# rrwick/Badread

Hardware: NVIDIA H100
Metric: simulated Gbases/sec (higher is better)
Workload: dtype u8/int32 (+f64 identity estimate)

## Files before the change

### badread_b200/csrc/bb_api.cu

```cuda
#include <cuda_runtime.h>
#include <dlfcn.h>
#include <unistd.h>

#include <algorithm>
#include <cstdio>
#include <cstdlib>
#include <cstring>
#include <memory>
#include <numeric>
#include <string>
#include <thread>
#include <vector>

#include "bb_kernels.cuh"
#include "bb_launch.h"

namespace {

struct DevBuf {
    void *p = nullptr;
    size_t cap = 0;
    DevBuf() = default;
    DevBuf(const DevBuf &) = delete;
    DevBuf &operator=(const DevBuf &) = delete;
// ... 640 lines not shown
    p.tbuf = w.s_tbuf.as<uint8_t>(); p.tbuf_stride = tbuf_stride;
    p.peq = w.s_peq.as<uint4>(); p.peq_stride = peq_cap; p.peq_cap = peq_cap;
    constexpr int lean_cap = 2048;
    const size_t lean_warps = (size_t)w.ctx->sm_count * kLeanCtasPerSmBoth * BB_WARPS_PER_CTA;
    BB_CUDA(&w, w.s_lr_lean.ensure(lean_warps * lean_cap * 2 * sizeof(int)));
    w.pool_lean = p;
    w.pool_lean.lr = w.s_lr_lean.as<int>(); w.pool_lean.lr_stride = 2ll * lean_cap; w.pool_lean.lr_cap = lean_cap;
    return BB_OK;
}

static BBBatchDev batch_dev(const Worker &w) {
    BBBatchDev B{};
    B.n_reads = w.n_reads;
    B.read_index = w.d_read_index.as<unsigned long long>();
    B.seg_off = w.d_seg_off.as<int>();
    B.segs = w.d_segs.as<bb_segment>();
    B.lit = w.d_lit.as<uint8_t>();
    B.target = w.d_target.as<double>();
    B.order = w.d_order.as<int>();
    B.reads = w.d_reads.as<BBReadDev>();
    B.frag = w.d_frag.as<uint8_t>();
    B.state = w.d_state.as<uint32_t>();
    B.kidx = w.d_kidx.as<int>();
    B.seq = w.d_seq.as<uint8_t>();
    B.ops = w.d_ops.as<uint8_t>();
    B.dcnt = w.d_dcnt.as<unsigned int>();
    B.qual = w.d_qual.as<uint8_t>();
    B.out_seq = w.d_out_seq.as<uint8_t>();
    B.out_qual = w.d_out_qual.as<uint8_t>();
    B.fpeq = w.d_fpeq.as<uint4>();
    B.speq = w.d_speq.as<uint4>();
    B.ctime = w.d_ctime.as<unsigned int>();
    B.chlog = w.d_chlog.as<uint2>();
    B.wres = w.d_wres.as<int2>();
    return B;
}

#define BB_N_COUNTERS 256
#define BB_ROUND_BASE(r) (16 + 16 * (r))
enum { BBC_MUTATE = 0, BBC_NTASKS = 1, BBC_LANE4 = 2, BBC_FB1 = 3, BBC_LANE8 = 4, BBC_FB2 = 5, BBC_WARP = 6, BBC_PENDING = 7 };

static int level_bound(int max_len, double slack) {
    long long mm = (long long)(max_len * slack) + 64;
    int d = 0;
    while (20ll * ((2 * mm + 64 + 63) / 64) * mm + 8ll * mm >= 1048576ll) { mm = (mm + 1) / 2; d++; }
    return d + 1;
}

static int w_prepare(Worker &w) {
    const bb_ctx &c = *w.ctx;
    BB_CUDA(&w, cudaSetDevice(c.device));
    Worker::Layout &L = w.L;
    const int n = w.n_reads;
    const int64_t off = w.frag_total;
    w.seq_cap = (int64_t)((double)off * w.slack) + 16ll * n + 65536;
    w.out_cap = w.seq_cap;
    w.speq_cap = w.seq_cap / 32 + (2ll * BB_PEQ_PAD + 2) * n + 64;
    L.fb_len = w.wres_total + 8;
    BB_CUDA(&w, w.d_frag.ensure((size_t)off + 16));
    BB_CUDA(&w, w.d_state.ensure(((size_t)off + 16) * sizeof(uint32_t)));
    BB_CUDA(&w, w.d_kidx.ensure(((size_t)off + 16) * sizeof(int)));
    BB_CUDA(&w, w.d_counter.ensure(BB_N_COUNTERS * sizeof(int)));
    BB_CUDA(&w, w.d_scan.ensure(sizeof(BBScanOut)));
    BB_CUDA(&w, w.d_levels.ensure(sizeof(Worker::RunInfo::levels)));
    BB_CUDA(&w, w.d_fpeq.ensure(((size_t)w.fpeq_total + 4) * sizeof(uint4)));
    BB_CUDA(&w, w.d_ctime.ensure(((size_t)off + 16) * sizeof(unsigned int)));
    BB_CUDA(&w, w.d_chlog.ensure(((size_t)w.log_total + 16) * sizeof(uint2)));
    BB_CUDA(&w, w.d_wres.ensure(((size_t)w.wres_total + 16) * sizeof(int2)));
    BB_CUDA(&w, w.d_wtasks.ensure(((size_t)w.wres_total + 16) * sizeof(BBWinTask)));
    BB_CUDA(&w, w.d_wfallback.ensure(2 * (size_t)L.fb_len * sizeof(BBWinTask)));
    BB_CUDA(&w, w.d_seq.ensure((size_t)w.seq_cap + 16));
    BB_CUDA(&w, w.d_ops.ensure((size_t)w.seq_cap + 16));
    BB_CUDA(&w, w.d_dcnt.ensure(((size_t)w.seq_cap + 16) * sizeof(unsigned int)));
    BB_CUDA(&w, w.d_qual.ensure((size_t)w.seq_cap + 16));
    BB_CUDA(&w, w.d_speq.ensure(((size_t)w.speq_cap + 4) * sizeof(uint4)));
    BB_CUDA(&w, w.d_out_seq.ensure((size_t)w.out_cap + 16));
    BB_CUDA(&w, w.d_out_qual.ensure((size_t)w.out_cap + 16));
    L.lane_ctas = c.sm_count * 4;
    const size_t lanes = (size_t)L.lane_ctas * 64;
    if (c.knobs.lowmem) {
        L.hist_per_pipe = lanes * BB_LEAF_MAX_TILES * BB_LEAF_CKPT_WORDS;
        BB_CUDA(&w, w.s_leafhist.ensure(2 * L.hist_per_pipe * sizeof(uint32_t)));
    } else {
        L.hist_per_pipe = lanes * BB_LEAF_LANE_COLS * BB_LEAF_LW;
        BB_CUDA(&w, w.s_lanehist.ensure(2 * L.hist_per_pipe * sizeof(uint2)));
    }
    BB_CUDA(&w, w.s_ltbuf.ensure(2 * lanes * BB_WIN_MAX_COLS));
    if (c.knobs.lowmem) BB_CUDA(&w, w.s_wckpt.ensure(2 * lanes * BB_WIN_MAX_TILES * BB_WIN_CKPT_WORDS(BB_WIN_LW) * sizeof(uint32_t)));
    const int len_b = (int)std::min<double>((double)w.max_len * w.slack + 64.0, (double)(1 << 24));
    const int lr_floor = c.knobs.lr_cap > 0 ? c.knobs.lr_cap : 4096;
    int lr_need = lr_floor;
    for (int r = 0; r < n; r++) {
        const double len = (double)w.h_reads[(size_t)r].frag_len;
        const double worst = len * w.slack + 64.0;
        const double expect = c.knobs.lr_cap > 0 ? 0.0 : 3.0 * (1.0 - w.h_target[(size_t)r]) * len + 0.02 * len + 512.0;
        lr_need = std::max(lr_need, (int)std::min(worst, w.lr_worst ? worst : expect));
    }
    int rc = ensure_scratch(w, len_b, lr_need, len_b, lr_floor);
    if (rc) return rc;
    int slot = 0;
    for (int s = 0; s < 2; s++)
        for (int k = 0; k < 3; k++) {
            L.lean_base[s][k] = slot;
            slot += c.sm_count * kLeanCtasPerSm[k] * BB_WARPS_PER_CTA;
        }
    L.cap_node = (int)std::min<int64_t>(w.seq_cap / 256 + 4ll * n + 1024, 0x7ffffff0);
    for (int s = 0; s < 2; s++) {
        auto &qb = w.qbuf[s];
        for (int k = 0; k < BBQ_NODE_CLASSES; k++)
            for (int p = 0; p < 2; p++) BB_CUDA(&w, qb.node[k][p].ensure((size_t)L.cap_node * sizeof(BBNode)));
        for (int x = 0; x < 2; x++) BB_CUDA(&w, qb.leaf[x].ensure((size_t)L.cap_node * sizeof(BBNode)));
        BB_CUDA(&w, qb.count.ensure(kQueueCounts * sizeof(int)));
    }
    w.n_levels = std::max(1, std::min(BB_MAX_LEVELS, level_bound(w.max_len, w.slack) + w.extra_levels));
    return BB_OK;
}

static int check_batch(bb_ctx *ctx, int32_t n_reads, const int32_t *seg_off, const bb_segment *segs, int64_t literal_len,
                       std::vector<int64_t> &len) {
    const int k = ctx->em.k;
    len.assign((size_t)n_reads, 0);
    for (int32_t r = 0; r < n_reads; r++) {
        if (seg_off[r + 1] < seg_off[r]) return set_err(ctx, BB_ERR_ARG, "seg_off must be non-decreasing");
        for (int32_t s = seg_off[r]; s < seg_off[r + 1]; s++) {
            const bb_segment &sg = segs[s];
            if (sg.len < 0 || sg.src < 0) return set_err(ctx, BB_ERR_ARG, "negative segment");
            if (sg.kind == BB_SEG_LITERAL) { if (sg.src + sg.len > literal_len) return set_err(ctx, BB_ERR_ARG, "literal segment out of range"); }
            else if (sg.kind == BB_SEG_REF_FWD || sg.kind == BB_SEG_REF_REV) { if (sg.src + sg.len > ctx->ref_len) return set_err(ctx, BB_ERR_ARG, "reference segment out of range"); }
            else return set_err(ctx, BB_ERR_ARG, "unknown segment kind");
            len[(size_t)r] += sg.len;
        }
        if (len[(size_t)r] + 2 * k >= (1 << 24)) return set_err(ctx, BB_ERR_ARG, "fragment too long (16 Mb limit)");
    }
    return BB_OK;
}

static int w_batch_upload(Worker &w, int32_t n_reads, const uint64_t *read_index, const int32_t *seg_off,
                          const bb_segment *segs, const uint8_t *literal_pool, int64_t literal_len,
                          const double *target_identity) {
    BB_CUDA(&w, cudaSetDevice(w.ctx->device));
    const int k = w.ctx->em.k;
    w.h_reads.assign((size_t)n_reads, BBReadDev{});
    w.h_inlen.assign((size_t)n_reads, 0);
    w.h_target.assign(target_identity, target_identity + n_reads);
    int64_t off = 0, peq_off = 0, log_off = 0, wres_off = 0;
    int max_len = 0;
    for (int32_t r = 0; r < n_reads; r++) {
        int64_t len = 0;
        for (int32_t s = seg_off[r]; s < seg_off[r + 1]; s++) len += segs[s].len;
        w.h_inlen[(size_t)r] = (int32_t)len;
        BBReadDev &rd = w.h_reads[(size_t)r];
        rd.frag_off = off;
        rd.frag_len = (int)(len + 2 * k);
        rd.fpeq_off = peq_off;
        peq_off += bb_peq_words(rd.frag_len);
        {
            const int cap = (int)(0.9 * (double)rd.frag_len) + k + 2;
            rd.log_off = log_off; rd.wres_off = wres_off;
            log_off += cap; wres_off += cap / BB_ALIGNMENT_INTERVAL + 1;
            const double need = (double)rd.frag_len * (1.0 - target_identity[r]);
            rd.horizon = (int)std::min<double>((double)cap, std::max(0.0, 1.25 * need) + 48.0);
            rd.n_logged = 0; rd.n_resume = 0; rd.a_done = 0; rd.status = BB_READ_PENDING; rd.stop_reason = 0;
        }
        off += (rd.frag_len + 15) & ~15;
        max_len = std::max(max_len, rd.frag_len);
    }
    w.frag_total = off; w.fpeq_total = peq_off; w.log_total = log_off; w.wres_total = wres_off;
// ... 1024 lines not shown
```

### badread_b200/csrc/bb_lane.cuh

```cuda
#pragma once
#include <cstdint>

#include "bb_align.cuh"

struct BBLaneProb {
    const uint4 *peq;
    int peq_bit0;
    const uint8_t *q;
    int n;
    const uint8_t *t;
    int m;
    int a, b;
    uint2 *hist;
};

__device__ __forceinline__ int bb_lane_words(int a, int b) { return ((a + b) >> 5) + 2; }

__device__ __forceinline__ void bb_lane_fetch(const BBLaneProb &P, int word, uint32_t &mA, uint32_t &mC, uint32_t &mG,
                                              uint32_t &mT) {
    mA = mC = mG = mT = 0u;
    const int R = word * 32;
    const int valid = P.n - R;
    if (valid <= 0) return;
    const int s = P.peq_bit0 + R;
    const int idx = s >> 5, sh = s & 31;
    const uint4 lo = P.peq[idx], hi = P.peq[idx + 1];
    mA = __funnelshift_r(lo.x, hi.x, sh); mC = __funnelshift_r(lo.y, hi.y, sh);
    mG = __funnelshift_r(lo.z, hi.z, sh); mT = __funnelshift_r(lo.w, hi.w, sh);
    if (valid < 32) {
        const uint32_t keep = (1u << valid) - 1u;
        mA &= keep; mC &= keep; mG &= keep; mT &= keep;
    }
}

template <int LW>
__device__ int bb_lane_pass(const BBLaneProb &P) {
    const int n = P.n, m = P.m, a = P.a;
    uint32_t Pv[LW], Mv[LW], eA[LW], eC[LW], eG[LW], eT[LW];
#pragma unroll
    for (int x = 0; x < LW; x++) {
        Pv[x] = ~0u; Mv[x] = 0u;
        bb_lane_fetch(P, x, eA[x], eC[x], eG[x], eT[x]);
    }
    int wt = 0;
    int score = 32 * LW;
    uint2 *h = P.hist;
    for (int c = 0; c < m; c++) {
        if (c - a >= 32 * (wt + 1)) {
#pragma unroll
            for (int x = 0; x + 1 < LW; x++) {
                Pv[x] = Pv[x + 1]; Mv[x] = Mv[x + 1];
                eA[x] = eA[x + 1]; eC[x] = eC[x + 1]; eG[x] = eG[x + 1]; eT[x] = eT[x + 1];
            }
            wt++;
            Pv[LW - 1] = ~0u; Mv[LW - 1] = 0u;
            bb_lane_fetch(P, wt + LW - 1, eA[LW - 1], eC[LW - 1], eG[LW - 1], eT[LW - 1]);
            score += 32;
        }
        const uint32_t tc = P.t[c];
        const uint32_t code = (tc >> 1) & 3u;
        const bool acgt = ((0x47544341u >> (8 * code)) & 0xffu) == tc;
        uint32_t Eq[LW], Xv[LW], A[LW], S[LW], Ph[LW], Mh[LW];
#pragma unroll
        for (int x = 0; x < LW; x++)
            Eq[x] = (code & 2u) ? ((code & 1u) ? eG[x] : eT[x]) : ((code & 1u) ? eC[x] : eA[x]);
        if (!acgt) {
#pragma unroll
            for (int x = 0; x < LW; x++) {
                Eq[x] = 0u;
                const int row0 = (wt + x) * 32;
                for (int r = 0; r < 32; r++)
                    if (row0 + r < n && P.q[row0 + r] == tc) Eq[x] |= 1u << r;
            }
        }
#pragma unroll
        for (int x = 0; x < LW; x++) { Xv[x] = Eq[x] | Mv[x]; A[x] = Eq[x] & Pv[x]; }
        bb_add_words<LW>(A, Pv, S);
#pragma unroll
        for (int x = 0; x < LW; x++) {
            const uint32_t Xh = (S[x] ^ Pv[x]) | Eq[x];
            Ph[x] = Mv[x] | ~(Xh | Pv[x]);
            Mh[x] = Pv[x] & Xh;
        }
        score += (int)(Ph[LW - 1] >> 31) - (int)(Mh[LW - 1] >> 31);
#pragma unroll
        for (int x = LW - 1; x >= 0; x--) {
            const uint32_t phs = __funnelshift_l(x > 0 ? Ph[x - 1] : 0x80000000u, Ph[x], 1);
            const uint32_t mhs = __funnelshift_l(x > 0 ? Mh[x - 1] : 0u, Mh[x], 1);
            const uint32_t raw = Ph[x];
            Pv[x] = mhs | ~(Xv[x] | phs);
            Mv[x] = phs & Xv[x];
            h[x] = make_uint2(Pv[x], raw);
        }
        h += LW;
    }
    int result = BB_INF;
    int run = score;
#pragma unroll
    for (int x = LW - 1; x >= 0; x--) {
        const int row0 = (wt + x) * 32;
        if (row0 <= n - 1 && n - 1 < row0 + 32) {
            const int bit = (n - 1) - row0;
            const uint32_t up = bit == 31 ? 0u : (Pv[x] >> (bit + 1));
            const uint32_t um = bit == 31 ? 0u : (Mv[x] >> (bit + 1));
            result = run - __popc(up) + __popc(um);
        }
        run -= __popc(Pv[x]) - __popc(Mv[x]);
    }
    return result;
}

template <int LW>
__device__ void bb_lane_traceback(const BBLaneProb &P, int &matches, int &dels, int &err) {
    const int a = P.a;
    int i = P.n - 1, j = P.m - 1;
    int mt = 0, dl = 0;
    while (i >= 0 && j >= 0) {
        int wt = (j - a) >> 5; if (wt < 0) wt = 0;
        const int x = (i >> 5) - wt;
        if (x < 0 || x >= LW) { err |= 1; break; }
        const uint2 e = P.hist[j * LW + x];
        const int bit = i & 31;
        if ((e.x >> bit) & 1u) { i--; }
        else if ((e.y >> bit) & 1u) { dl++; j--; }
        else { mt += (P.q[i] == P.t[j]) ? 1 : 0; i--; j--; }
    }
    if (j >= 0) dl += j + 1;
    matches = mt; dels = dl;
}

template <int LW>
__device__ __forceinline__ void bb_prefetch_history(const uint2 *hist, int tj) {
#if defined(__CUDA_ARCH__)
    const long long e = (long long)tj * LW;
    if ((e & 15) == 0 && e >= 48) asm volatile("prefetch.global.L2 [%0];" ::"l"(hist + (e - 48)));
#endif
}

#define BB_RING_BYTES(LW, T) (2 * (T) * (LW) * 64 * 8)

__device__ __forceinline__ void bb_cp_async8(uint2 *smem, const uint2 *gmem) {
#if defined(__CUDA_ARCH__)
    asm volatile("cp.async.ca.shared.global [%0], [%1], 8;" ::"r"((uint32_t)__cvta_generic_to_shared(smem)), "l"(gmem) : "memory");
#else
    *smem = *gmem;
#endif
}
__device__ __forceinline__ void bb_cp_async_commit() {
#if defined(__CUDA_ARCH__)
    asm volatile("cp.async.commit_group;" ::: "memory");
#endif
}
template <int N>
__device__ __forceinline__ void bb_cp_async_wait() {
#if defined(__CUDA_ARCH__)
    asm volatile("cp.async.wait_group %0;" ::"n"(N) : "memory");
#endif
}

template <int LW, int T>
__device__ __forceinline__ void bb_ring_tick(uint2 *ring, const uint2 *hist, int tj, int &staged_lo) {
    const bool fresh = staged_lo > tj;
    if (fresh) {
        const int lo1 = max(0, tj - T + 1);
        for (int col = tj; col >= lo1; col--) {
#pragma unroll
            for (int x = 0; x < LW; x++) bb_cp_async8(ring + ((col & (2 * T - 1)) * LW + x) * 64, hist + (long long)col * LW + x);
        }
        bb_cp_async_commit();
        staged_lo = lo1;
    }
    const int want_lo = max(0, tj - 2 * T + 1);
    for (int col = staged_lo - 1; col >= want_lo; col--) {
#pragma unroll
        for (int x = 0; x < LW; x++) bb_cp_async8(ring + ((col & (2 * T - 1)) * LW + x) * 64, hist + (long long)col * LW + x);
    }
    bb_cp_async_commit();
    if (want_lo < staged_lo) staged_lo = want_lo;
#if defined(__CUDA_ARCH__)
    {
        constexpr int LINES = (T * LW * 8 + 127) / 128 + 1;
        const long long e = ((long long)tj - 4 * T) * LW;
#pragma unroll
        for (int x = 0; x < 2 * LINES; x++)
            if (e + 16 * x >= 0 && (x < LINES || fresh)) asm volatile("prefetch.global.L2 [%0];" ::"l"(hist + e + 16 * x));
    }
#endif
    bb_cp_async_wait<1>();
}

template <int LW, int T>
__device__ __forceinline__ uint2 bb_ring_entry(const uint2 *ring, int col, int x) {
    return ring[((col & (2 * T - 1)) * LW + x) * 64];
}
```

### badread_b200/csrc/bb_loop.cuh

```cuda
#pragma once
#include <cstdint>

#include "bb_lane.cuh"

enum { BB_STOP_HORIZON = 0, BB_STOP_LIMIT = 1, BB_STOP_COUNT = 2, BB_STOP_NOLOOP = 3 };

#define BB_WIN_LW 8
#define BB_WIN_MAX_COLS 2048

struct BBWinTask { int r, a; };

#define BB_MUTP_THREADS (BB_WARPS_PER_CTA * 32 + 32)

template <int BB_TU_ = 0>
__global__ void __launch_bounds__(BB_MUTP_THREADS)
bb_k_mutate(BBBatchDev B, BBErrorModelDev em, unsigned long long seed, int *work_counter, const int *order,
                 int n_items) {
    constexpr int NE = BB_WARPS_PER_CTA * 32;
    __shared__ int s_kind[2][NE], s_pos[2][NE], s_rpos[2][NE];
    __shared__ uint32_t s_pay[2][NE];
    __shared__ int s_w, s_stop, s_cc;
    __shared__ long long s_n0;
    const int lane = threadIdx.x & 31;
    const int warp = threadIdx.x >> 5;
// ... 343 lines not shown
            if (tm > BB_WIN_MAX_COLS || bb_lane_words(P.a, P.b) > LW || !bb_uses_traceback(qn, tm)) {
                fallback[atomicAdd(fallback_count, 1)] = tk;
                active = false;
            }
        }
        if (!active) tm = 0;
        BBLanePass<LW> S;
        if (active) {
            P.n = qn; P.peq = B.fpeq + rd->fpeq_off; P.q = frag + qpos; P.qs = 1;
            P.peq_bit0 = qpos + BB_PEQ_BIT0; P.t = tbuf; P.ts = 1;
            bb_lane_begin<LW>(S, P);
        }
        const int tm_max = __reduce_max_sync(BB_FULL, tm);
        for (int c = 0; c < tm_max; c++) {
            if (c < tm) {
                if ((c & (BB_WIN_TILE - 1)) == 0) {
                    uint32_t *ck = ckpt + (c / BB_WIN_TILE) * CKW;
#pragma unroll
                    for (int x = 0; x < LW; x++) { ck[x] = S.Pv[x]; ck[LW + x] = S.Mv[x]; }
                    ck[2 * LW] = (uint32_t)S.wt; ck[2 * LW + 1] = (uint32_t)S.score;
                }
                bb_lane_step<LW, false>(S, P, nullptr);
            }
        }
        int ti = qn - 1, tj = tm - 1, matches = 0, dels = 0;
        bool walking = active && ti >= 0 && tj >= 0;
        bool need_tile = walking;
        int tile_lo = 0;
        for (int round = 0; round < 2 * BB_WIN_MAX_COLS + 64 && __any_sync(BB_FULL, walking); round++) {
            if (walking && need_tile) {
                const int tile = tj / BB_WIN_TILE;
                tile_lo = tile * BB_WIN_TILE;
                const uint32_t *ck = ckpt + tile * CKW;
#pragma unroll
                for (int x = 0; x < LW; x++) { S.Pv[x] = ck[x]; S.Mv[x] = ck[LW + x]; }
                S.wt = (int)ck[2 * LW]; S.score = (int)ck[2 * LW + 1]; S.c = tile_lo;
#pragma unroll
                for (int x = 0; x < LW; x++) bb_fetch_peq(P, 32 * (S.wt + x), S.eA[x], S.eC[x], S.eG[x], S.eT[x]);
                const int hi = min(tile_lo + BB_WIN_TILE, tm);
                for (int c = tile_lo; c < hi; c++) bb_lane_step<LW, true, 64>(S, P, hs + ((c - tile_lo) * LW) * 64);
                need_tile = false;
            }
            for (int mv = 0; mv < 64; mv++) {
                const bool can = walking && !need_tile;
                if (!__any_sync(BB_FULL, can)) break;
                if (can) {
                    int wt = (tj - P.a) >> 5; if (wt < 0) wt = 0;
                    const int x = (ti >> 5) - wt;
                    if (x < 0 || x >= LW) { atomicOr(&B.reads[tk.r].flags, 1); ti = -1; tj = -1; }
                    else {
                        const uint2 e = hs[((tj - tile_lo) * LW + x) * 64];
                        const int bit = ti & 31;
                        if ((e.x >> bit) & 1u) ti--;
                        else if ((e.y >> bit) & 1u) { dels++; tj--; }
                        else { matches += (frag[qpos + ti] == tbuf[tj]) ? 1 : 0; ti--; tj--; }
                    }
                    if (ti < 0 || tj < 0) walking = false;
                    else if (tj < tile_lo) need_tile = true;
                }
            }
        }
        if (active) {
            if (walking) atomicOr(&B.reads[tk.r].flags, 1);
            if (tj >= 0) dels += tj + 1;
            B.wres[rd->wres_off + tk.a - 1] = make_int2(matches, qn + dels);
        }
    }
}

#ifndef BB_WIN_RING_T
#define BB_WIN_RING_T 4
#endif
template <int LW, int T = BB_WIN_RING_T>
__global__ void __launch_bounds__(64, (LW <= 4 ? 8 : 4))
bb_k_window_lane_hist(BBBatchDev B, BBErrorModelDev em, const BBWinTask *tasks, const int *n_tasks_ptr, unsigned long long seed,
                 uint2 *hist_pool, uint8_t *tbuf_pool, int *cursor, BBWinTask *fallback, int *fallback_count) {
#ifdef BB_EMULATOR
    static uint2 s_ring[BB_RING_BYTES(LW, T) / 8];
#else
    extern __shared__ __align__(16) uint2 s_ring[];
#endif
    const int n_tasks = *n_tasks_ptr;
    const long long gl = (long long)blockIdx.x * blockDim.x + threadIdx.x;
    uint2 *const hist = hist_pool + gl * (long long)(BB_WIN_MAX_COLS * LW);
    uint8_t *const tbuf = tbuf_pool + gl * (long long)BB_WIN_MAX_COLS;
    uint2 *const ring = s_ring + threadIdx.x;
    BBLanePass<LW> S;
    BBProb P;
    BBWinTask tk = {0, 0};
    const uint8_t *frag = nullptr;
    const uint32_t *state = nullptr;
    const unsigned int *ctime = nullptr;
    int phase = 0;
    int qpos = 0, qn = 0, jx = 0, tm = 0, uw = 0, ti = 0, tj = 0, diags = 0, dels = 0, dist = 0, staged_lo = 0;
    unsigned int tmax = 0;
    for (;;) {
        if (phase == 0) {
            const int w = atomicAdd(cursor, 1);
            if (w >= n_tasks) phase = 4;
            else {
                tk = tasks[w];
                const BBReadDev *rd = &B.reads[tk.r];
                frag = B.frag + rd->frag_off; state = B.state + rd->frag_off; ctime = B.ctime + rd->frag_off;
                bb_window_of(rd->frag_len, seed, B.read_index[tk.r], tk.a, qpos, qn);
                tmax = (unsigned int)(BB_ALIGNMENT_INTERVAL * tk.a);
                jx = 0; tm = 0; uw = 0;
                phase = 1;
            }
        }
        if (__all_sync(BB_FULL, phase == 4)) break;
        for (int it = 0; it < 64; it++) {
            if (phase == 1) {
                unsigned int ct4[4];
                uint8_t fb4[4];
#pragma unroll
                for (int h = 0; h < 4; h++) {
                    const int j = min(jx + h, qn - 1);
                    ct4[h] = ctime[qpos + j];
                    fb4[h] = frag[qpos + j];
                }
#pragma unroll
                for (int h = 0; h < 4; h++) {
                    if (jx < qn) {
                        if (ct4[h] == 0u || ct4[h] > tmax) { if (tm < BB_WIN_MAX_COLS) tbuf[tm] = fb4[h]; tm++; }
                        else {
                            const uint32_t st = state[qpos + jx];
                            const int sl = (int)(st & 0xff);
                            for (int c = 0; c < sl; c++) { if (tm < BB_WIN_MAX_COLS) tbuf[tm] = bb_slot_char(em, st, c); tm++; }
                            uw += sl < 1 ? 1 : sl;
                        }
                        jx++;
                    }
                }
                if (jx >= qn) {
                    const int diff = qn > tm ? qn - tm : tm - qn;
                    if (uw < diff) uw = diff;
                    const int mx = qn > tm ? qn : tm;
                    if (uw > mx) uw = mx;
                    bb_band(qn, tm, uw, P.a, P.b);
                    if (tm > BB_WIN_MAX_COLS || bb_lane_words(P.a, P.b) > LW || !bb_uses_traceback(qn, tm)) {
                        fallback[atomicAdd(fallback_count, 1)] = tk;
                        phase = 0;
                    } else {
                        const BBReadDev *rd = &B.reads[tk.r];
                        P.n = qn; P.peq = B.fpeq + rd->fpeq_off; P.q = frag + qpos; P.qs = 1;
                        P.peq_bit0 = qpos + BB_PEQ_BIT0; P.t = tbuf; P.ts = 1;
                        bb_lane_begin<LW>(S, P);
                        phase = 2;
                    }
                }
            }
        }
        for (int it = 0; it < 128; it++) {
            if (phase == 2) {
                bb_lane_step<LW, true>(S, P, hist + (long long)S.c * LW);
                if (S.c >= tm) {
                    dist = bb_lane_corner<LW>(S, qn);
                    ti = qn - 1; tj = tm - 1; diags = 0; dels = 0; staged_lo = tm; phase = 3;
                }
            }
        }
        for (int it = 0; it < 256; it++) {
            if (phase == 3) {
                if (ti >= 0 && tj >= 0) {
                    if ((it & (T - 1)) == 0) bb_ring_tick<LW, T>(ring, hist, tj, staged_lo);
                    int wt = (tj - P.a) >> 5; if (wt < 0) wt = 0;
                    const int x = (ti >> 5) - wt;
                    if (x < 0 || x >= LW) { atomicOr(&B.reads[tk.r].flags, 1); ti = -1; tj = -1; }
                    else {
                        const uint2 e = bb_ring_entry<LW, T>(ring, tj, x);
                        const int bit = ti & 31;
                        if ((e.x >> bit) & 1u) ti--;
                        else if ((e.y >> bit) & 1u) { dels++; tj--; }
                        else { diags++; ti--; tj--; }
                    }
                } else {
                    bb_cp_async_wait<0>();
                    if (tj >= 0) dels += tj + 1;
                    const int matches = diags - (dist - (qn - diags) - dels);
                    if (dist >= BB_INF) atomicOr(&B.reads[tk.r].flags, 1);
                    B.wres[B.reads[tk.r].wres_off + tk.a - 1] = make_int2(matches, qn + dels);
                    phase = 0;
                }
            }
        }
    }
}

template <int BB_TU_ = 0>
__global__ void __launch_bounds__(BB_WARPS_PER_CTA * 32, 4)
bb_k_window_warp(BBBatchDev B, BBErrorModelDev em, BBScratchPool pool, const BBWinTask *tasks, const int *n_tasks_ptr,
                 unsigned long long seed, int *cursor) {
    const int lane = threadIdx.x & 31;
    const int warp = blockIdx.x * BB_WARPS_PER_CTA + (threadIdx.x >> 5);
    BBScratch sc = pool.for_warp(warp);
    uint8_t *tbuf = pool.tbuf + (long long)warp * pool.tbuf_stride;
    const int n_tasks = *n_tasks_ptr;
    BBEmit no_emit = {nullptr, nullptr, nullptr};
    for (;;) {
        int w = 0;
        if (lane == 0) w = atomicAdd(cursor, 1);
        w = __shfl_sync(BB_FULL, w, 0);
        if (w >= n_tasks) break;
        const BBWinTask tk = tasks[w];
        BBReadDev *rd = &B.reads[tk.r];
        const uint8_t *frag = B.frag + rd->frag_off;
        const uint32_t *state = B.state + rd->frag_off;
        const unsigned int *ctime = B.ctime + rd->frag_off;
        int qpos, qn;
        bb_window_of(rd->frag_len, seed, B.read_index[tk.r], tk.a, qpos, qn);
        const unsigned int tmax = (unsigned int)(BB_ALIGNMENT_INTERVAL * tk.a);
        int total = 0, up = 0;
        for (int base = 0; base < qn; base += 32) {
            const int x = base + lane;
            uint32_t st = BB_SLOT_NONE;
            int len = 0;
            if (x < qn) {
                const unsigned int ct = ctime[qpos + x];
                if (ct != 0u && ct <= tmax) st = state[qpos + x];
                len = st == BB_SLOT_NONE ? 1 : (int)(st & 0xff);
            }
            int incl = len;
#pragma unroll
            for (int d = 1; d < 32; d <<= 1) {
                const int v = __shfl_up_sync(BB_FULL, incl, d);
                if (lane >= d) incl += v;
            }
            const int off = total + incl - len;
            if (x < qn) {
                if (st == BB_SLOT_NONE) tbuf[off] = frag[qpos + x];
                else {
                    for (int c = 0; c < len; c++) tbuf[off + c] = bb_slot_char(em, st, c);
                    up += len < 1 ? 1 : len;
                }
            }
            total += __shfl_sync(BB_FULL, incl, 31);
        }
#pragma unroll
        for (int d = 16; d > 0; d >>= 1) up += __shfl_xor_sync(BB_FULL, up, d);
        __syncwarp();
        sc.peq = B.fpeq + rd->fpeq_off;
        BBAlnCounts cnt = {0, 0, 0, 0};
        bb_align<false, 1>(frag + qpos, qn, tbuf, total, up, sc, no_emit, qpos, cnt);
        __syncwarp();
        if (lane == 0) {
            if (cnt.err) atomicOr(&rd->flags, cnt.err);
            B.wres[rd->wres_off + tk.a - 1] = make_int2(cnt.matches, qn + cnt.dels);
        }
        __syncwarp();
    }
}

template <int BB_TU_ = 0>
__global__ void __launch_bounds__(128)
// ... 87 lines not shown
```

### badread_b200/csrc/bb_tasks.cuh

```cuda
#pragma once
#include <cstdint>

#include "bb_align.cuh"
#include "bb_lane.cuh"

#define BB_NODE_LW_SMALL 8
#define BB_LEAF_LW 8
#define BB_LEAF_LANE_COLS 2048

enum { BBQ_NODE_LANE8 = 0, BBQ_NODE_LEAN1 = 1, BBQ_NODE_LEAN2 = 2, BBQ_NODE_LEAN4 = 3, BBQ_NODE_WIDE = 4, BBQ_NODE_CLASSES = 5 };
#define BBQ_COUNT(cls, parity) ((parity) * BBQ_NODE_CLASSES + (cls))
#define BBQ_LEAF_COUNT 10
#define BBQ_OVERFLOW 12
#define BBQ_BACKWARDS 2

struct BBNode { int r, q0, nn, t0, mm, best; };

struct BBQueues {
    BBNode *node[BBQ_NODE_CLASSES][2];
    BBNode *leaf[2];
    int *count;
    int *overflow;
    int cap_node, cap_leaf;
    int lane8_cols;
// ... 76 lines not shown
    }
    return false;
}

template <int BB_TU_ = 0>
__global__ void __launch_bounds__(256) bb_k_push_roots(BBBatchDev B, BBQueues QN, BBQueues QW, const int *order) {
    const int i = blockIdx.x * blockDim.x + threadIdx.x;
    if (i >= B.n_reads) return;
    const int r = order[i];
    BBReadDev *rd = &B.reads[r];
    if (rd->flags & BB_FLAG_NOSPACE) return;
    BBAlignOut o;
    o.ops = B.ops + rd->seq_off; o.dcnt = B.dcnt + rd->seq_off; o.rd = rd;
    const BBNode nd = {r, 0, rd->seq_len, 0, rd->frag_len, -1};
    int a, b;
    bb_task_band(nd, rd->upper, a, b);
    const bool wide = !bb_uses_traceback(nd.nn, nd.mm) && bb_pick_L<4>(a, b, 16) == 0;
    bb_push_task(wide ? QW : QN, 0, o, nd, rd->upper);
}

template <int LW>
struct BBLanePass {
    uint32_t Pv[LW], Mv[LW], eA[LW], eC[LW], eG[LW], eT[LW];
    int wt, score, c;
};

template <int LW>
__device__ __forceinline__ void bb_lane_begin(BBLanePass<LW> &S, const BBProb &P) {
#pragma unroll
    for (int x = 0; x < LW; x++) {
        S.Pv[x] = ~0u; S.Mv[x] = 0u;
        bb_fetch_peq(P, 32 * x, S.eA[x], S.eC[x], S.eG[x], S.eT[x]);
    }
    S.wt = 0; S.score = 32 * LW; S.c = 0;
}

template <int LW, bool HIST, int HSTRIDE = 1>
__device__ __forceinline__ void bb_lane_step(BBLanePass<LW> &S, const BBProb &P, uint2 *hist) {
    const int c = S.c;
    if (c - P.a >= 32 * (S.wt + 1)) {
#pragma unroll
        for (int x = 0; x + 1 < LW; x++) {
            S.Pv[x] = S.Pv[x + 1]; S.Mv[x] = S.Mv[x + 1];
            S.eA[x] = S.eA[x + 1]; S.eC[x] = S.eC[x + 1]; S.eG[x] = S.eG[x + 1]; S.eT[x] = S.eT[x + 1];
        }
        S.wt++;
        S.Pv[LW - 1] = ~0u; S.Mv[LW - 1] = 0u;
        bb_fetch_peq(P, 32 * (S.wt + LW - 1), S.eA[LW - 1], S.eC[LW - 1], S.eG[LW - 1], S.eT[LW - 1]);
        S.score += 32;
    }
    const uint32_t tc = P.t[(long long)c * P.ts];
    const uint32_t code = (tc >> 1) & 3u;
    const bool acgt = ((0x47544341u >> (8 * code)) & 0xffu) == tc;
    uint32_t Eq[LW], Xv[LW], A[LW], Sm[LW], Ph[LW], Mh[LW];
#pragma unroll
    for (int x = 0; x < LW; x++)
        Eq[x] = (code & 2u) ? ((code & 1u) ? S.eG[x] : S.eT[x]) : ((code & 1u) ? S.eC[x] : S.eA[x]);
    if (!acgt) {
#pragma unroll
        for (int x = 0; x < LW; x++) {
            Eq[x] = 0u;
            const int row0 = (S.wt + x) * 32;
            for (int r = 0; r < 32; r++)
                if (row0 + r < P.n && P.q[(long long)(row0 + r) * P.qs] == tc) Eq[x] |= 1u << r;
        }
    }
#pragma unroll
    for (int x = 0; x < LW; x++) { Xv[x] = Eq[x] | S.Mv[x]; A[x] = Eq[x] & S.Pv[x]; }
    bb_add_words<LW>(A, S.Pv, Sm);
#pragma unroll
    for (int x = 0; x < LW; x++) {
        const uint32_t Xh = (Sm[x] ^ S.Pv[x]) | Eq[x];
        Ph[x] = S.Mv[x] | ~(Xh | S.Pv[x]);
        Mh[x] = S.Pv[x] & Xh;
    }
    S.score += (int)(Ph[LW - 1] >> 31) - (int)(Mh[LW - 1] >> 31);
#pragma unroll
    for (int x = LW - 1; x >= 0; x--) {
        const uint32_t phs = __funnelshift_l(x > 0 ? Ph[x - 1] : 0x80000000u, Ph[x], 1);
        const uint32_t mhs = __funnelshift_l(x > 0 ? Mh[x - 1] : 0u, Mh[x], 1);
        const uint32_t raw = Ph[x];
        S.Pv[x] = mhs | ~(Xv[x] | phs);
        S.Mv[x] = phs & Xv[x];
        if (HIST && (HSTRIDE != 1 || (LW & 1))) hist[x * HSTRIDE] = make_uint2(S.Pv[x], raw);
        if (HIST && HSTRIDE == 1 && !(LW & 1)) Ph[x] = raw;
    }
    if (HIST && HSTRIDE == 1 && !(LW & 1)) {
#pragma unroll
        for (int x = 0; x < LW; x += 2)
            reinterpret_cast<uint4 *>(hist)[x >> 1] = make_uint4(S.Pv[x], Ph[x], S.Pv[x + 1], Ph[x + 1]);
    }
    S.c = c + 1;
}

template <int LW>
__device__ int bb_lane_column_scores(const BBLanePass<LW> &S, int n, int lo, int hi, int *out) {
    int result = BB_INF;
    int run = S.score;
#pragma unroll
    for (int x = LW - 1; x >= 0; x--) {
        const int row0 = (S.wt + x) * 32;
        int rr = run;
        for (int r = 31; r >= 0; r--) {
            const int row = row0 + r;
            if (row < n) {
                if (out && row >= lo && row <= hi) out[row - lo] = rr;
                if (row == n - 1) result = rr;
            }
            rr -= (int)((S.Pv[x] >> r) & 1u) - (int)((S.Mv[x] >> r) & 1u);
        }
        run -= __popc(S.Pv[x]) - __popc(S.Mv[x]);
    }
    return result;
}

template <int LW>
__device__ __forceinline__ int bb_lane_corner(const BBLanePass<LW> &S, int n) {
    int result = BB_INF;
    int run = S.score;
#pragma unroll
    for (int x = LW - 1; x >= 0; x--) {
        const int row0 = (S.wt + x) * 32;
        if (row0 <= n - 1 && n - 1 < row0 + 32) {
            const int bit = (n - 1) - row0;
            const uint32_t up = bit == 31 ? 0u : (S.Pv[x] >> (bit + 1));
            const uint32_t um = bit == 31 ? 0u : (S.Mv[x] >> (bit + 1));
            result = run - __popc(up) + __popc(um);
        }
        run -= __popc(S.Pv[x]) - __popc(S.Mv[x]);
    }
    return result;
}

template <int LW>
__global__ void __launch_bounds__(64, 6)
bb_k_node_lane(BBBatchDev B, BBQueues Q, int parity_order, int *cursor) {
    constexpr int CLS = BBQ_NODE_LANE8;
    const int parity = parity_order & 1;
    const bool backwards = (parity_order & BBQ_BACKWARDS) != 0;
    const BBNode *list = Q.node[CLS][parity];
    const int count = min(Q.count[BBQ_COUNT(CLS, parity)], Q.cap_node);
    BBLanePass<LW> S;
    BBProb P;
    BBNode nd;
    int Lc[32 * LW], Rc[32 * LW];
    int loL = 0, hiL = 0, loR = 0, hiR = 0, left_w = 0, right_w = 0, ncols = 0, upper = 0;
    int phase = 0;
    BBAlignOut o;
    for (;;) {
        if (phase == 0) {
            const int w = atomicAdd(cursor, 1);
            if (w >= count) phase = 3;
            else {
                nd = list[backwards ? count - 1 - w : w];
                BBReadDev *rd = &B.reads[nd.r];
                o.ops = B.ops + rd->seq_off; o.dcnt = B.dcnt + rd->seq_off; o.rd = rd;
                upper = rd->upper;
                bb_task_band(nd, upper, P.a, P.b);
                left_w = nd.mm / 2; right_w = nd.mm - left_w;
                loL = max(0, left_w - 1 - P.a); hiL = min(nd.nn - 1, left_w - 1 + P.b);
                loR = max(0, right_w - 1 - P.a); hiR = min(nd.nn - 1, right_w - 1 + P.b);
                P.n = nd.nn; P.peq = B.speq + rd->speq_off;
                P.q = B.seq + rd->seq_off + nd.q0; P.qs = 1; P.peq_bit0 = nd.q0 + BB_PEQ_BIT0;
                P.t = B.frag + rd->frag_off + nd.t0; P.ts = 1;
                ncols = left_w;
                bb_lane_begin<LW>(S, P);
                phase = 1;
            }
        }
        if (__all_sync(BB_FULL, phase == 3)) break;
        for (int it = 0; it < 128; it++) {
            if (phase == 1 || phase == 2) {
                bb_lane_step<LW, false>(S, P, nullptr);
// ... 69 lines not shown
        for (int c = 0; c < mm_max; c++) {
            if (c < mm) {
                if ((c & (BB_LEAF_TILE - 1)) == 0) {
                    uint32_t *ck = ckpt + (c / BB_LEAF_TILE) * CKW;
#pragma unroll
                    for (int x = 0; x < LW; x++) { ck[x] = S.Pv[x]; ck[LW + x] = S.Mv[x]; }
                    ck[2 * LW] = (uint32_t)S.wt; ck[2 * LW + 1] = (uint32_t)S.score;
                }
                bb_lane_step<LW, false>(S, P, nullptr);
            }
        }
        if (active) {
            const int d = bb_lane_column_scores<LW>(S, nd.nn, 0, -1, nullptr);
            if (nd.best >= 0 && d != nd.best) atomicOr(&o.rd->flags, 8 << 8);
        }
        int ti = nd.nn - 1, tj = mm - 1, matches = 0, dels = 0;
        bool walking = active && ti >= 0 && tj >= 0;
        bool need_tile = walking;
        int tile_lo = 0;
        for (int round = 0; round < (1 << 16) && __any_sync(BB_FULL, walking); round++) {
            if (walking && need_tile) {
                const int tile = tj / BB_LEAF_TILE;
                tile_lo = tile * BB_LEAF_TILE;
                const uint32_t *ck = ckpt + tile * CKW;
#pragma unroll
                for (int x = 0; x < LW; x++) { S.Pv[x] = ck[x]; S.Mv[x] = ck[LW + x]; }
                S.wt = (int)ck[2 * LW]; S.score = (int)ck[2 * LW + 1]; S.c = tile_lo;
#pragma unroll
                for (int x = 0; x < LW; x++) bb_fetch_peq(P, 32 * (S.wt + x), S.eA[x], S.eC[x], S.eG[x], S.eT[x]);
                const int hi = min(tile_lo + BB_LEAF_TILE, mm);
                for (int c = tile_lo; c < hi; c++) bb_lane_step<LW, true, 64>(S, P, hs + ((c - tile_lo) * LW) * 64);
                need_tile = false;
            }
            for (int mv = 0; mv < 64; mv++) {
                const bool can = walking && !need_tile;
                if (!__any_sync(BB_FULL, can)) break;
                if (can) {
                    int wt = (tj - P.a) >> 5; if (wt < 0) wt = 0;
                    const int x = (ti >> 5) - wt;
                    if (x < 0 || x >= LW) { atomicOr(&o.rd->flags, 1 << 8); ti = -1; tj = -1; }
                    else {
                        const uint2 e = hs[((tj - tile_lo) * LW + x) * 64];
                        const int bit = ti & 31;
                        if ((e.x >> bit) & 1u) { o.ops[nd.q0 + ti] = BB_OP_I; ti--; }
                        else if ((e.y >> bit) & 1u) { bb_add_dels(o, nd.q0 + ti, 1); dels++; tj--; }
                        else {
                            const bool eq = qp[ti] == tp[tj];
                            o.ops[nd.q0 + ti] = eq ? BB_OP_EQ : BB_OP_X;
                            matches += eq ? 1 : 0;
                            ti--; tj--;
                        }
                    }
                    if (ti < 0 || tj < 0) walking = false;
                    else if (tj < tile_lo) need_tile = true;
                }
            }
        }
        if (active) {
            if (walking) atomicOr(&o.rd->flags, 1 << 8);
            for (int x = 0; x <= ti; x++) o.ops[nd.q0 + x] = BB_OP_I;
            if (tj >= 0) { bb_add_dels(o, nd.q0 - 1, tj + 1); dels += tj + 1; }
            atomicAdd(&o.rd->matches, matches);
            atomicAdd(&o.rd->dels, dels);
        }
    }
}

#ifndef BB_LEAF_RING_T
#define BB_LEAF_RING_T 4
#endif
#define BB_LEAF_RING_BYTES BB_RING_BYTES(BB_LEAF_LW, BB_LEAF_RING_T)

template <int BB_TU_ = 0>
__global__ void __launch_bounds__(64)
bb_k_leaf_lane_hist(BBBatchDev B, BBQueues Q, uint2 *hist_pool, int *cursor) {
    constexpr int LW = BB_LEAF_LW, T = BB_LEAF_RING_T;
#ifdef BB_EMULATOR
    static uint2 s_ring[BB_LEAF_RING_BYTES / 8];
#else
    extern __shared__ __align__(16) uint2 s_ring[];
#endif
    const BBNode *list = Q.leaf[0];
    const int count = min(Q.count[BBQ_LEAF_COUNT], Q.cap_leaf);
    uint2 *const hist = hist_pool + ((long long)blockIdx.x * blockDim.x + threadIdx.x) * (long long)(BB_LEAF_LANE_COLS * LW);
    uint2 *const ring = s_ring + threadIdx.x;
    BBLanePass<LW> S;
    BBProb P;
    BBNode nd;
    BBAlignOut o;
    const uint8_t *qp = nullptr, *tp = nullptr;
    int phase = 0;
    int ti = 0, tj = 0, matches = 0, dels = 0, staged_lo = 0;
    for (;;) {
        if (phase == 0) {
            const int w = atomicAdd(cursor, 1);
            if (w >= count) phase = 3;
            else {
                nd = list[w];
                BBReadDev *rd = &B.reads[nd.r];
                o.ops = B.ops + rd->seq_off; o.dcnt = B.dcnt + rd->seq_off; o.rd = rd;
                bb_task_band(nd, rd->upper, P.a, P.b);
                P.n = nd.nn; P.peq = B.speq + rd->speq_off;
                qp = B.seq + rd->seq_off + nd.q0; tp = B.frag + rd->frag_off + nd.t0;
                P.q = qp; P.qs = 1; P.peq_bit0 = nd.q0 + BB_PEQ_BIT0; P.t = tp; P.ts = 1;
                bb_lane_begin<LW>(S, P);
                phase = 1;
            }
        }
        if (__all_sync(BB_FULL, phase == 3)) break;
        for (int it = 0; it < 128; it++) {
            if (phase == 1) {
                bb_lane_step<LW, true>(S, P, hist + (long long)S.c * LW);
                if (S.c >= nd.mm) {
                    const int d = bb_lane_corner<LW>(S, nd.nn);
                    if (nd.best >= 0 && d != nd.best) atomicOr(&o.rd->flags, 8 << 8);
                    ti = nd.nn - 1; tj = nd.mm - 1; matches = 0; dels = 0; staged_lo = nd.mm;
                    phase = 2;
                }
            }
        }
        for (int it = 0; it < 256; it++) {
            if (phase == 2) {
                if (ti >= 0 && tj >= 0) {
                    if ((it & (T - 1)) == 0) bb_ring_tick<LW, T>(ring, hist, tj, staged_lo);
                    int wt = (tj - P.a) >> 5; if (wt < 0) wt = 0;
                    const int x = (ti >> 5) - wt;
                    if (x < 0 || x >= LW) { atomicOr(&o.rd->flags, 1 << 8); ti = -1; tj = -1; }
                    else {
                        const uint2 e = bb_ring_entry<LW, T>(ring, tj, x);
                        const int bit = ti & 31;
                        if ((e.x >> bit) & 1u) { o.ops[nd.q0 + ti] = BB_OP_I; ti--; }
                        else if ((e.y >> bit) & 1u) { bb_add_dels(o, nd.q0 + ti, 1); dels++; tj--; }
                        else {
                            const bool eq = qp[ti] == tp[tj];
                            o.ops[nd.q0 + ti] = eq ? BB_OP_EQ : BB_OP_X;
                            matches += eq ? 1 : 0;
                            ti--; tj--;
                        }
                    }
                } else {
                    bb_cp_async_wait<0>();
                    for (int x = 0; x <= ti; x++) o.ops[nd.q0 + x] = BB_OP_I;
                    if (tj >= 0) { bb_add_dels(o, nd.q0 - 1, tj + 1); dels += tj + 1; }
                    atomicAdd(&o.rd->matches, matches);
                    atomicAdd(&o.rd->dels, dels);
                    phase = 0;
                }
            }
        }
    }
}

template <int L>
__global__ void __launch_bounds__(BB_WARPS_PER_CTA * 32, (L == 1 ? 6 : L == 2 ? 5 : 3))
bb_k_node_warp(BBBatchDev B, BBQueues Q, BBScratchPool pool, int parity_order, int *cursor, int warp_base) {
    constexpr int CLS = L == 1 ? BBQ_NODE_LEAN1 : L == 2 ? BBQ_NODE_LEAN2 : BBQ_NODE_LEAN4;
    const int parity = parity_order & 1;
    const bool backwards = (parity_order & BBQ_BACKWARDS) != 0;
    const int lane = threadIdx.x & 31;
    const int warp = warp_base + blockIdx.x * BB_WARPS_PER_CTA + (threadIdx.x >> 5);
    BBScratch sc = pool.for_warp(warp);
    const BBNode *list = Q.node[CLS][parity];
    const int count = min(Q.count[BBQ_COUNT(CLS, parity)], Q.cap_node);
    for (;;) {
        int w = 0;
        if (lane == 0) w = atomicAdd(cursor, 1);
        w = __shfl_sync(BB_FULL, w, 0);
        if (w >= count) break;
        const BBNode nd = list[backwards ? count - 1 - w : w];
        BBReadDev *rd = &B.reads[nd.r];
        BBAlignOut o;
        o.ops = B.ops + rd->seq_off; o.dcnt = B.dcnt + rd->seq_off; o.rd = rd;
        sc.peq = B.speq + rd->speq_off;
        const uint8_t *q = B.seq + rd->seq_off, *t = B.frag + rd->frag_off;
        int a, b;
        bb_task_band(nd, rd->upper, a, b);
        const int left_w = nd.mm / 2, right_w = nd.mm - left_w;
        const int loL = max(0, left_w - 1 - a), hiL = min(nd.nn - 1, left_w - 1 + b);
        const int loR = max(0, right_w - 1 - a), hiR = min(nd.nn - 1, right_w - 1 + b);
        int best = nd.best, split = 0, ls = 0, rs = 0, err = 0;
        if (hiL - loL + 1 > sc.lr_cap || hiR - loR + 1 > sc.lr_cap) err = 16;
        else {
            BBProb P;
            P.n = nd.nn; P.a = a; P.b = b; P.peq = sc.peq; P.hist = nullptr; P.nb_alloc = 0;
            P.tpeq = B.fpeq + rd->fpeq_off;
            if (lane < 16) {
                P.q = q + nd.q0; P.qs = 1; P.t = t + nd.t0; P.ts = 1; P.ncols = left_w;
                P.peq_bit0 = nd.q0 + BB_PEQ_BIT0; P.cols_out = sc.L; P.cols_lo = loL;
                P.tpeq_bit0 = nd.t0 + BB_PEQ_BIT0;
            } else {
                P.q = q + nd.q0 + nd.nn - 1; P.qs = -1; P.t = t + nd.t0 + nd.mm - 1; P.ts = -1; P.ncols = right_w;
                P.peq_bit0 = nd.q0 + nd.nn - 1 + BB_PEQ_BIT0; P.cols_out = sc.R; P.cols_lo = loR;
                P.tpeq_bit0 = nd.t0 + nd.mm - 1 + BB_PEQ_BIT0;
            }
            bb_band_pass_bp<L>(P, 16);
            __syncwarp();
            err = bb_split_warp(sc, loL, hiL, loR, hiR, nd.nn, left_w, right_w, best, split, ls, rs);
        }
        __syncwarp();
        if (lane == 0) {
            if (err) atomicOr(&rd->flags, err << 8);
            else {
                BBNode c0 = {nd.r, nd.q0, split + 1, nd.t0, left_w, ls};
                BBNode c1 = {nd.r, nd.q0 + split + 1, nd.nn - split - 1, nd.t0 + left_w, right_w, rs};
                bb_push_task(Q, parity ^ 1, o, c0, rd->upper);
                bb_push_task(Q, parity ^ 1, o, c1, rd->upper);
            }
        }
        __syncwarp();
    }
}

#define BB_PAIR_SMEM_BYTES (BB_WARPS_PER_CTA * bb_esm_words(32) * 4)
// ... 212 lines not shown
```

Before: 1.100.

## Store band-aligned traceback history with only the needed words per column

The per-column history now holds only the band's words (bw = (a+b)/32+1, at most LW-1). Each column is funnel-shifted so it starts at the band's lower edge, rather than storing all LW tile words. Traceback indexes by the offset within the band, and the cp.async ring, prefetch and global pool sizes shrink to match. This cuts global history write and read traffic and shared-memory ring size, at the cost of extra funnel shifts per column and a runtime bound on the store loops.

```diff
diff --git a/badread_b200/csrc/bb_api.cu b/badread_b200/csrc/bb_api.cu
--- a/badread_b200/csrc/bb_api.cu
+++ b/badread_b200/csrc/bb_api.cu
@@ -746,7 +746,7 @@
         L.hist_per_pipe = lanes * BB_LEAF_MAX_TILES * BB_LEAF_CKPT_WORDS;
         BB_CUDA(&w, w.s_leafhist.ensure(2 * L.hist_per_pipe * sizeof(uint32_t)));
     } else {
-        L.hist_per_pipe = lanes * BB_LEAF_LANE_COLS * BB_LEAF_LW;
+        L.hist_per_pipe = lanes * BB_LEAF_LANE_COLS * (BB_LEAF_LW - 1);
         BB_CUDA(&w, w.s_lanehist.ensure(2 * L.hist_per_pipe * sizeof(uint2)));
     }
     BB_CUDA(&w, w.s_ltbuf.ensure(2 * lanes * BB_WIN_MAX_COLS));
diff --git a/badread_b200/csrc/bb_lane.cuh b/badread_b200/csrc/bb_lane.cuh
--- a/badread_b200/csrc/bb_lane.cuh
+++ b/badread_b200/csrc/bb_lane.cuh
@@ -15,6 +15,7 @@
 };
 
 __device__ __forceinline__ int bb_lane_words(int a, int b) { return ((a + b) >> 5) + 2; }
+__device__ __forceinline__ int bb_band_words(int a, int b) { return ((a + b) >> 5) + 1; }
 
 __device__ __forceinline__ void bb_lane_fetch(const BBLaneProb &P, int word, uint32_t &mA, uint32_t &mC, uint32_t &mG,
                                               uint32_t &mT) {
@@ -137,7 +138,7 @@
 #endif
 }
 
-#define BB_RING_BYTES(LW, T) (2 * (T) * (LW) * 64 * 8)
+#define BB_RING_BYTES(LW, T) (2 * (T) * ((LW) - 1) * 64 * 8)
 
 __device__ __forceinline__ void bb_cp_async8(uint2 *smem, const uint2 *gmem) {
 #if defined(__CUDA_ARCH__)
@@ -158,14 +159,15 @@
 #endif
 }
 
-template <int LW, int T>
-__device__ __forceinline__ void bb_ring_tick(uint2 *ring, const uint2 *hist, int tj, int &staged_lo) {
+template <int RW, int T>
+__device__ __forceinline__ void bb_ring_tick(uint2 *ring, const uint2 *hist, int bw, int tj, int &staged_lo) {
     const bool fresh = staged_lo > tj;
     if (fresh) {
         const int lo1 = max(0, tj - T + 1);
         for (int col = tj; col >= lo1; col--) {
 #pragma unroll
-            for (int x = 0; x < LW; x++) bb_cp_async8(ring + ((col & (2 * T - 1)) * LW + x) * 64, hist + (long long)col * LW + x);
+            for (int x = 0; x < RW; x++)
+                if (x < bw) bb_cp_async8(ring + ((col & (2 * T - 1)) * RW + x) * 64, hist + (long long)col * bw + x);
         }
         bb_cp_async_commit();
         staged_lo = lo1;
@@ -173,23 +175,25 @@
     const int want_lo = max(0, tj - 2 * T + 1);
     for (int col = staged_lo - 1; col >= want_lo; col--) {
 #pragma unroll
-        for (int x = 0; x < LW; x++) bb_cp_async8(ring + ((col & (2 * T - 1)) * LW + x) * 64, hist + (long long)col * LW + x);
+        for (int x = 0; x < RW; x++)
+            if (x < bw) bb_cp_async8(ring + ((col & (2 * T - 1)) * RW + x) * 64, hist + (long long)col * bw + x);
     }
     bb_cp_async_commit();
     if (want_lo < staged_lo) staged_lo = want_lo;
 #if defined(__CUDA_ARCH__)
     {
-        constexpr int LINES = (T * LW * 8 + 127) / 128 + 1;
-        const long long e = ((long long)tj - 4 * T) * LW;
+        constexpr int MAX_LINES = (T * RW * 8 + 127) / 128 + 1;
+        const int lines = (T * bw * 8 + 127) / 128 + 1;
+        const long long e = ((long long)tj - 4 * T) * bw;
 #pragma unroll
-        for (int x = 0; x < 2 * LINES; x++)
-            if (e + 16 * x >= 0 && (x < LINES || fresh)) asm volatile("prefetch.global.L2 [%0];" ::"l"(hist + e + 16 * x));
+        for (int x = 0; x < 2 * MAX_LINES; x++)
+            if (e + 16 * x >= 0 && x < (fresh ? 2 : 1) * lines) asm volatile("prefetch.global.L2 [%0];" ::"l"(hist + e + 16 * x));
     }
 #endif
     bb_cp_async_wait<1>();
 }
 
-template <int LW, int T>
+template <int RW, int T>
 __device__ __forceinline__ uint2 bb_ring_entry(const uint2 *ring, int col, int x) {
-    return ring[((col & (2 * T - 1)) * LW + x) * 64];
+    return ring[((col & (2 * T - 1)) * RW + x) * 64];
 }
diff --git a/badread_b200/csrc/bb_loop.cuh b/badread_b200/csrc/bb_loop.cuh
--- a/badread_b200/csrc/bb_loop.cuh
+++ b/badread_b200/csrc/bb_loop.cuh
@@ -449,7 +449,7 @@
 #endif
     const int n_tasks = *n_tasks_ptr;
     const long long gl = (long long)blockIdx.x * blockDim.x + threadIdx.x;
-    uint2 *const hist = hist_pool + gl * (long long)(BB_WIN_MAX_COLS * LW);
+    uint2 *const hist = hist_pool + gl * (long long)(BB_WIN_MAX_COLS * (LW - 1));
     uint8_t *const tbuf = tbuf_pool + gl * (long long)BB_WIN_MAX_COLS;
     uint2 *const ring = s_ring + threadIdx.x;
     BBLanePass<LW> S;
@@ -459,7 +459,7 @@
     const uint32_t *state = nullptr;
     const unsigned int *ctime = nullptr;
     int phase = 0;
-    int qpos = 0, qn = 0, jx = 0, tm = 0, uw = 0, ti = 0, tj = 0, diags = 0, dels = 0, dist = 0, staged_lo = 0;
+    int qpos = 0, qn = 0, jx = 0, tm = 0, uw = 0, ti = 0, tj = 0, diags = 0, dels = 0, dist = 0, staged_lo = 0, bw = 1;
     unsigned int tmax = 0;
     for (;;) {
         if (phase == 0) {
@@ -513,6 +513,7 @@
                         P.n = qn; P.peq = B.fpeq + rd->fpeq_off; P.q = frag + qpos; P.qs = 1;
                         P.peq_bit0 = qpos + BB_PEQ_BIT0; P.t = tbuf; P.ts = 1;
                         bb_lane_begin<LW>(S, P);
+                        bw = bb_band_words(P.a, P.b);
                         phase = 2;
                     }
                 }
@@ -520,7 +521,7 @@
         }
         for (int it = 0; it < 128; it++) {
             if (phase == 2) {
-                bb_lane_step<LW, true>(S, P, hist + (long long)S.c * LW);
+                bb_lane_step<LW, true>(S, P, hist + (long long)S.c * bw);
                 if (S.c >= tm) {
                     dist = bb_lane_corner<LW>(S, qn);
                     ti = qn - 1; tj = tm - 1; diags = 0; dels = 0; staged_lo = tm; phase = 3;
@@ -530,13 +531,12 @@
         for (int it = 0; it < 256; it++) {
             if (phase == 3) {
                 if (ti >= 0 && tj >= 0) {
-                    if ((it & (T - 1)) == 0) bb_ring_tick<LW, T>(ring, hist, tj, staged_lo);
-                    int wt = (tj - P.a) >> 5; if (wt < 0) wt = 0;
-                    const int x = (ti >> 5) - wt;
-                    if (x < 0 || x >= LW) { atomicOr(&B.reads[tk.r].flags, 1); ti = -1; tj = -1; }
+                    if ((it & (T - 1)) == 0) bb_ring_tick<LW - 1, T>(ring, hist, bw, tj, staged_lo);
+                    const int k = ti - max(0, tj - P.a);
+                    if (k < 0 || k >= 32 * bw) { atomicOr(&B.reads[tk.r].flags, 1); ti = -1; tj = -1; }
                     else {
-                        const uint2 e = bb_ring_entry<LW, T>(ring, tj, x);
-                        const int bit = ti & 31;
+                        const uint2 e = bb_ring_entry<LW - 1, T>(ring, tj, k >> 5);
+                        const int bit = k & 31;
                         if ((e.x >> bit) & 1u) ti--;
                         else if ((e.y >> bit) & 1u) { dels++; tj--; }
                         else { diags++; ti--; tj--; }
diff --git a/badread_b200/csrc/bb_tasks.cuh b/badread_b200/csrc/bb_tasks.cuh
--- a/badread_b200/csrc/bb_tasks.cuh
+++ b/badread_b200/csrc/bb_tasks.cuh
@@ -182,13 +182,14 @@
         const uint32_t raw = Ph[x];
         S.Pv[x] = mhs | ~(Xv[x] | phs);
         S.Mv[x] = phs & Xv[x];
-        if (HIST && (HSTRIDE != 1 || (LW & 1))) hist[x * HSTRIDE] = make_uint2(S.Pv[x], raw);
-        if (HIST && HSTRIDE == 1 && !(LW & 1)) Ph[x] = raw;
-    }
-    if (HIST && HSTRIDE == 1 && !(LW & 1)) {
-#pragma unroll
-        for (int x = 0; x < LW; x += 2)
-            reinterpret_cast<uint4 *>(hist)[x >> 1] = make_uint4(S.Pv[x], Ph[x], S.Pv[x + 1], Ph[x + 1]);
+        if (HIST && HSTRIDE != 1) hist[x * HSTRIDE] = make_uint2(S.Pv[x], raw);
+    }
+    if (HIST && HSTRIDE == 1) {
+        const int bw = bb_band_words(P.a, P.b);
+        const int off = c >= P.a ? (c - P.a) & 31 : 0;
+#pragma unroll
+        for (int y = 0; y + 1 < LW; y++)
+            if (y < bw) hist[y] = make_uint2(__funnelshift_r(S.Pv[y], S.Pv[y + 1], off), __funnelshift_r(Ph[y], Ph[y + 1], off));
     }
     S.c = c + 1;
 }
@@ -424,7 +425,7 @@
 #endif
     const BBNode *list = Q.leaf[0];
     const int count = min(Q.count[BBQ_LEAF_COUNT], Q.cap_leaf);
-    uint2 *const hist = hist_pool + ((long long)blockIdx.x * blockDim.x + threadIdx.x) * (long long)(BB_LEAF_LANE_COLS * LW);
+    uint2 *const hist = hist_pool + ((long long)blockIdx.x * blockDim.x + threadIdx.x) * (long long)(BB_LEAF_LANE_COLS * (LW - 1));
     uint2 *const ring = s_ring + threadIdx.x;
     BBLanePass<LW> S;
     BBProb P;
@@ -452,7 +453,7 @@
         if (__all_sync(BB_FULL, phase == 3)) break;
         for (int it = 0; it < 128; it++) {
             if (phase == 1) {
-                bb_lane_step<LW, true>(S, P, hist + (long long)S.c * LW);
+                bb_lane_step<LW, true>(S, P, hist + (long long)S.c * bb_band_words(P.a, P.b));
                 if (S.c >= nd.mm) {
                     const int d = bb_lane_corner<LW>(S, nd.nn);
                     if (nd.best >= 0 && d != nd.best) atomicOr(&o.rd->flags, 8 << 8);
@@ -464,13 +465,13 @@
         for (int it = 0; it < 256; it++) {
             if (phase == 2) {
                 if (ti >= 0 && tj >= 0) {
-                    if ((it & (T - 1)) == 0) bb_ring_tick<LW, T>(ring, hist, tj, staged_lo);
-                    int wt = (tj - P.a) >> 5; if (wt < 0) wt = 0;
-                    const int x = (ti >> 5) - wt;
-                    if (x < 0 || x >= LW) { atomicOr(&o.rd->flags, 1 << 8); ti = -1; tj = -1; }
+                    const int bw = bb_band_words(P.a, P.b);
+                    if ((it & (T - 1)) == 0) bb_ring_tick<LW - 1, T>(ring, hist, bw, tj, staged_lo);
+                    const int k = ti - max(0, tj - P.a);
+                    if (k < 0 || k >= 32 * bw) { atomicOr(&o.rd->flags, 1 << 8); ti = -1; tj = -1; }
                     else {
-                        const uint2 e = bb_ring_entry<LW, T>(ring, tj, x);
-                        const int bit = ti & 31;
+                        const uint2 e = bb_ring_entry<LW - 1, T>(ring, tj, k >> 5);
+                        const int bit = k & 31;
                         if ((e.x >> bit) & 1u) { o.ops[nd.q0 + ti] = BB_OP_I; ti--; }
                         else if ((e.y >> bit) & 1u) { bb_add_dels(o, nd.q0 + ti, 1); dels++; tj--; }
                         else {
```

Result: faster. 1.183 (median of 6 runs) (+7.6%).
